# youngers2006/Dreamer

Hardware: AMD Instinct MI355X
Metric: imagined latent-steps/sec (B×H) at 64×64 CarRacing, 1/2/4/8 MI355X (higher is better)
Workload: dtype f32; 1 GPU; Dreamer.train_Agent() with AC_epochs=1 (replay sample + warm start S/2 + H-step imagination + actor-critic update), B=256/GPU S=64 H=15 64x64x3, precision=fp32 (north-star batch per GPU); global_batch=256, seq_len=64, horizon=15, parallelism=dp1, precision=fp32

## Files before the change

dreamer_amd/csrc/gemm.hip:

```cpp
#include <limits.h>
#include <stdlib.h>
#include <stdint.h>
#include <string.h>

#include "gemm.h"

#include <algorithm>

#define BK 32
#define LDS_K (BK + 2)

struct GemmBatch {
  GemmArgs p[4];
};

template <int BM, int BN>
__device__ __forceinline__ int dr_pack_tile(const GemmBatch& gb, int npack, int& z) {
  z = blockIdx.z;
  if (npack <= 0) return -2;
  int tot = 0;
  for (int i = 0; i < npack; ++i) tot += ((gb.p[i].M + BM - 1) / BM) * ((gb.p[i].N + BN - 1) / BN);
  int lt = dr_xcd_tile(blockIdx.x, tot);
  if (lt < 0) return -1;
  z = 0;
// ... 167 lines not shown
    if (!B_KN) {
      const int kk = tid & 31, nb = tid >> 5;
#pragma unroll
      for (int i = 0; i < NB; ++i) Bs[nb + 8 * i][kk] = rb[i];
    } else {
      const int nl = tid % BN, kb = tid / BN;
#pragma unroll
      for (int i = 0; i < NB; ++i) Bs[nl][kb + (256 / BN) * i] = rb[i];
    }
  };

  constexpr int WAVES_M = (BM >= 32) ? 2 : 1, WAVES_N = 4 / WAVES_M;
  constexpr int WTM = BM / WAVES_M, WTN = BN / WAVES_N;
  constexpr int FM = WTM / 16, FN = WTN / 16;
  static_assert(FM >= 1 && FN >= 1, "tile too small for 4 waves");
  const int wm0 = (wave / WAVES_N) * WTM, wn0 = (wave % WAVES_N) * WTN;
  f32x4 acc[FM][FN];
#pragma unroll
  for (int i = 0; i < FM; ++i)
#pragma unroll
    for (int j = 0; j < FN; ++j) acc[i][j] = (f32x4){0.f, 0.f, 0.f, 0.f};

  const int fr = lane & 15, fk = lane >> 4;
  load_tiles(0);
  for (int k0 = 0; k0 < K; k0 += BK) {
    __syncthreads();
    store_tiles();
    __syncthreads();
    if (k0 + BK < K) load_tiles(k0 + BK);
#pragma unroll
    for (int kk = 0; kk < BK; kk += 4) {
      float a[FM], b[FN];
#pragma unroll
      for (int i = 0; i < FM; ++i) a[i] = As[wm0 + i * 16 + fr][kk + fk];
#pragma unroll
      for (int j = 0; j < FN; ++j) b[j] = Bs[wn0 + j * 16 + fr][kk + fk];
#pragma unroll
      for (int i = 0; i < FM; ++i)
#pragma unroll
        for (int j = 0; j < FN; ++j) acc[i][j] = __builtin_amdgcn_mfma_f32_16x16x4f32(a[i], b[j], acc[i][j], 0, 0, 0);
    }
  }

#pragma unroll
  for (int i = 0; i < FM; ++i)
#pragma unroll
    for (int j = 0; j < FN; ++j)
#pragma unroll
      for (int r = 0; r < 4; ++r) {
        const int m = m0 + wm0 + i * 16 + fk * 4 + r;
        const int n = n0 + wn0 + j * 16 + fr;
        if (m >= M || n >= N) continue;
        float v = (g.alpha == 1.0f) ? acc[i][j][r] : g.alpha * acc[i][j][r];
        if (g.bias) v = v + g.bias[n];
        if (g.addend) v = v + g.addend[(long long)m * g.ld_add + n];
        if (g.act == 1) v = v / (1.0f + expf(-v));
        else if (g.act == 2) v = 1.0f / (1.0f + expf(-v));
        float* dst;
        if (g.out_conv) {
          const int hw = g.oh * g.ow;
          const int f = m / hw, pix = m - f * hw;
          dst = g.Y + ((long long)f * N + n) * hw + pix;
        } else if (n < g.nsplitY) {
          dst = g.Y + (long long)m * g.ldy + n;
        } else {
          dst = g.Y2 + (long long)m * g.ldy2 + (n - g.nsplitY);
        }
        if (g.accumulate) *dst = *dst + v;
        else *dst = v;
      }
}

#ifdef DR_PHASE_TIMING
__device__ long long dr_tbuf_gemm[1024 * DR_TS_SLOTS];
extern "C" int dr_debug_tbuf_gemm(long long* out, int n) {
  const int rc = (int)hipMemcpyFromSymbol(out, HIP_SYMBOL(dr_tbuf_gemm), (size_t)n * sizeof(long long));
  static long long zeros[1024 * DR_TS_SLOTS];
  return rc | (int)hipMemcpyToSymbol(HIP_SYMBOL(dr_tbuf_gemm), zeros, sizeof(zeros));
}
#endif
#define SK_LN_MAXF 33280
#define SK_LN_MAXK 2048
#define SK_STAGE 8

struct SkOps {
  const float *A, *A2, *W, *W2;
  int lda, lda2, ksA, ldb, ldb2, ksB, nsB, M, N, K;
};

template <bool B_KN, bool VEC>
__device__ __forceinline__ void skinny_load_b(const SkOps& o, int n, int kq, float (&b)[4]) {
  if (!B_KN && VEC) {
    const bool ok = (n < o.N) && (kq < o.K);
    float4 v = dr_ld4(o.W, ok ? (unsigned)(n * o.ldb + kq) : 0u);
    if (!ok) v = make_float4(0.f, 0.f, 0.f, 0.f);
    b[0] = v.x; b[1] = v.y; b[2] = v.z; b[3] = v.w;
    return;
  }
#pragma unroll
  for (int c = 0; c < 4; ++c) {
    const int k = kq + c;
    const bool ok = (n < o.N) && (k < o.K);
    float v;
    if (!B_KN) {
      v = dr_ld1(o.W, ok ? (unsigned)(n * o.ldb + k) : 0u);
    } else if (k >= o.ksB) {
      v = dr_ld1(o.W2, ok ? (unsigned)((k - o.ksB) * o.ldb2 + n) : 0u);
    } else if (n >= o.nsB) {
      v = dr_ld1(o.W2, ok ? (unsigned)(k * o.ldb2 + n - o.nsB) : 0u);
    } else {
      v = dr_ld1(o.W, ok ? (unsigned)(k * o.ldb + n) : 0u);
    }
    b[c] = ok ? v : 0.f;
  }
}

template <bool VEC>
__device__ __forceinline__ void skinny_load_a(const SkOps& o, int m, int k16, int kq, float (&a)[4]) {
  if (VEC) {
    const bool ok = (m < o.M) && (kq < o.K);
    float4 v;
    if (k16 + 16 <= o.ksA) {
      v = dr_ld4(o.A, ok ? (unsigned)(m * o.lda + kq) : 0u);
    } else if (k16 >= o.ksA) {
      v = dr_ld4(o.A2, ok ? (unsigned)(m * o.lda2 + kq - o.ksA) : 0u);
    } else {
      const float* src = (kq < o.ksA) ? o.A + (long long)m * o.lda + kq : o.A2 + (long long)m * o.lda2 + (kq - o.ksA);
      v = dr_ld4(ok ? src : o.A, 0u);
    }
    if (!ok) v = make_float4(0.f, 0.f, 0.f, 0.f);
    a[0] = v.x; a[1] = v.y; a[2] = v.z; a[3] = v.w;
  } else {
#pragma unroll
    for (int c = 0; c < 4; ++c) {
      const int k = kq + c;
      const bool ok = (m < o.M) && (k < o.K);
      float v;
      if (k < o.ksA) v = dr_ld1(o.A, ok ? (unsigned)(m * o.lda + k) : 0u);
      else v = dr_ld1(o.A2, ok ? (unsigned)(m * o.lda2 + k - o.ksA) : 0u);
      a[c] = ok ? v : 0.f;
    }
  }
}

__device__ __forceinline__ float epi_act(const GemmArgs& g, float v) {
  if (g.act == 1) return v / (1.0f + expf(-v));
  if (g.act == 2) return 1.0f / (1.0f + expf(-v));
  return v;
}

__device__ __noinline__ void gru_bwd_elem(const GruBwdEpi& e, int m, int j, float g) {
  const int Hd = e.Hd;
  const long long i = (long long)m * Hd + j;
  const float r = dr_g(e.r)[i], u = dr_g(e.u)[i], n = dr_g(e.n)[i], hn = dr_g(e.ghn)[i];
  const float hv = e.h ? dr_g(e.h)[(long long)m * e.ldh + j] : 0.0f;
  const float g_hmn = g * u;
  const float g_u = g * (hv - n);
  const float g_n = g + (-g_hmn);
  const float g_pn = g_n * (1.0f - n * n);
  const float g_r = g_pn * hn;
  const float g_hn = g_pn * r;
  const float g_pr = g_r * (1.0f - r) * r;
  const float g_pu = g_u * (1.0f - u) * u;
  DR_GLOBAL float* gib = dr_g(e.gi) + (long long)m * 3 * Hd;
  DR_GLOBAL float* ghb = dr_g(e.gh) + (long long)m * 3 * Hd;
  gib[j] = g_pr;
  gib[Hd + j] = g_pu;
  gib[2 * Hd + j] = g_pn;
  ghb[j] = g_pr;
  ghb[Hd + j] = g_pu;
  ghb[2 * Hd + j] = g_hn;
  if (e.gi16) {
    DR_GLOBAL unsigned short* gi16 = dr_g(e.gi16) + (long long)m * 3 * Hd;
    DR_GLOBAL unsigned short* gh16 = dr_g(e.gh16) + (long long)m * 3 * Hd;
    gi16[j] = __builtin_bit_cast(unsigned short, (__bf16)g_pr);
    gi16[Hd + j] = __builtin_bit_cast(unsigned short, (__bf16)g_pu);
    gi16[2 * Hd + j] = __builtin_bit_cast(unsigned short, (__bf16)g_pn);
    gh16[j] = __builtin_bit_cast(unsigned short, (__bf16)g_pr);
    gh16[Hd + j] = __builtin_bit_cast(unsigned short, (__bf16)g_pu);
    gh16[2 * Hd + j] = __builtin_bit_cast(unsigned short, (__bf16)g_hn);
  }
  DR_GLOBAL float* o = dr_g(e.ho) + (long long)m * e.ldo + j;
  *o = *o + g_hmn;
}

__device__ __forceinline__ void epilogue_store_b(const GemmArgs& g, int m, int n, float acc, float bias) {
  float v = (g.alpha == 1.0f) ? acc : g.alpha * acc;
  if (g.bias) v = v + bias;
  if (g.addend) v = v + dr_g(g.addend)[(long long)m * g.ld_add + n];
  v = epi_act(g, v);
  DR_GLOBAL float* dst;
  if (n < g.nsplitY) dst = dr_g(g.Y) + (long long)m * g.ldy + n;
  else dst = dr_g(g.Y2) + (long long)m * g.ldy2 + (n - g.nsplitY);
  const float fin = g.accumulate ? *dst + v : v;
  *dst = fin;
  if (g.gb.Hd > 0 && n < g.gb.Hd) gru_bwd_elem(g.gb, m, n, fin);
}

#define DR_SKW 8
template <int MT, int NT, int AMODE, bool B_KN, bool VEC, int EPI>
__global__ __launch_bounds__(64 * DR_SKW) void k_gemm_skinny(GemmBatch gb, int npack) {
  constexpr int NWAVE = DR_SKW, NTH = 64 * DR_SKW, FT = MT / 16, FN = NT / 16;
  __shared__ GemmArgs s_args;
  int pz;
  const int plt = dr_pack_tile<MT, NT>(gb, npack, pz);
  if (plt == -1) return;
  dr_stage_args(gb.p[pz], s_args, threadIdx.x);
  const GemmArgs& g = s_args;
  SkOps o;
  o.M = dr_uni(g.M); o.N = dr_uni(g.N); o.K = dr_uni(g.K);
  o.A = dr_uni(g.A); o.A2 = dr_uni(g.A2); o.W = dr_uni(g.W);
  o.lda = dr_uni((int)g.lda); o.lda2 = dr_uni((int)g.lda2); o.ksA = dr_uni(g.ksplitA); o.ldb = dr_uni((int)g.ldb);
  o.W2 = dr_uni(g.W2); o.ldb2 = dr_uni((int)g.ldb2); o.ksB = dr_uni(g.ksplitB); o.nsB = dr_uni(g.nsplitB);
  const int M = o.M, N = o.N, K = o.K;
  const int tiles_n = (N + NT - 1) / NT;
  const int tiles_m = (M + MT - 1) / MT;
  const int lt = plt >= 0 ? plt : dr_xcd_tile(blockIdx.x, tiles_m * tiles_n);
  if (lt < 0) return;
  const int tn = lt / tiles_m, tm = lt - tn * tiles_m;
  const int m0 = tm * MT, n0 = tn * NT;
  const int tid = threadIdx.x, wave = tid >> 6, lane = tid & 63;
  const int r = lane & 15, q = lane >> 4;
  DR_TS(dr_tbuf_gemm, 0);

  constexpr int RED = NWAVE * FT * FN * 4 * 64;
  extern __shared__ __attribute__((aligned(16))) float smem[];
  __shared__ float s_mean[MT], s_rstd[MT];
  __shared__ float s_out[MT][NT + 1];
  constexpr int NEPI = (FT * FN * 256 + NTH - 1) / NTH;
  float ebias[NEPI];
  {
    const float* bias = dr_uni(g.bias);
#pragma unroll
    for (int i = 0; i < NEPI; ++i) {
      const int x = tid + NTH * i;
      const int n = n0 + ((x >> 8) % FN) * 16 + (x & 15);
      const bool ok = bias && x < FT * FN * 256 && n < N;
      const float v = dr_ld1(ok ? bias : o.W, ok ? (unsigned)n : 0u);
      ebias[i] = ok ? v : 0.f;
    }
  }

  unsigned long long rng_seed = 0, rng_off = 0;
  if ((EPI == EPI_SAMPLE || EPI == EPI_ACTOR) && g.epi != EPI_NONE && !g.noise.q && !g.noise.eps && g.noise.rng) {
    rng_seed = g.noise.rng[0];
    rng_off = g.noise.rng[1];
  }
  const int kw = ((K + NWAVE * 16 - 1) / (NWAVE * 16)) * 16;
  const int kb = wave * kw;
  const int ke = min(K, kb + kw);

  const int KP = K + ((8 - (K & 15)) & 15);
  const int K4 = K >> 2;
  constexpr int RPW = MT / NWAVE;
  constexpr int BPW = (NT + NWAVE - 1) / NWAVE;
  constexpr int SV = (MT == 16) ? 4 : 1;
  float* a_out = dr_uni(g.a_out);
  const int ld_aout = dr_uni((int)g.ld_aout);
  const bool store_a = (a_out != nullptr) && (tn == 0);
  const bool staged = (AMODE == AM_LNSILU || AMODE == AM_LNBWD || AMODE == AM_STEBWD) && VEC && !B_KN &&
                     (K4 <= 64 * SV) &&
                     ((MT + NT) * KP <= SK_LN_MAXF);
  constexpr bool DUAL = FT * FN < 4;
  f32x4 acc[FT][FN], acc2[FT][FN];
#pragma unroll
  for (int t = 0; t < FT; ++t)
#pragma unroll
    for (int j = 0; j < FN; ++j) acc[t][j] = acc2[t][j] = (f32x4){0.f, 0.f, 0.f, 0.f};
  DR_TS(dr_tbuf_gemm, 1);
  if (staged) {
    float* sA = smem;
    float* sB = smem + MT * KP;
    constexpr int PRW = (AMODE == AM_LNBWD || AMODE == AM_STEBWD) ? RPW : 1;
    float4 xa[RPW][SV], xb[BPW][SV], gv[SV], bv[SV], xp[PRW][SV];
    const float* lg = dr_uni(g.ln_g);
    const float* lb = dr_uni(g.ln_b);
    const float* pre = dr_uni(g.pre);
    const int ld_pre = dr_uni((int)g.ld_pre);
#pragma unroll
    for (int i = 0; i < SV; ++i) {
      if (64 * i >= K4) break;
      const int k4 = lane + 64 * i, k = 4 * k4;
      const bool okk = k4 < K4;
#pragma unroll
      for (int rr = 0; rr < RPW; ++rr) {
        const int m = m0 + wave + NWAVE * rr;
        const bool ok = okk && m < M;
        const bool seg1 = k < o.ksA;
        const float* base = seg1 ? o.A : o.A2;
        const unsigned e = ok ? (unsigned)(seg1 ? m * o.lda + k : m * o.lda2 + k - o.ksA) : 0u;
        xa[rr][i] = dr_ld4(ok ? base : o.W, e);
        if (!ok) xa[rr][i] = make_float4(0.f, 0.f, 0.f, 0.f);
        if (AMODE == AM_LNBWD || AMODE == AM_STEBWD) {
          xp[rr][i] = dr_ld4(pre, ok ? (unsigned)(m * ld_pre + k) : 0u);
          if (!ok) xp[rr][i] = make_float4(0.f, 0.f, 0.f, 0.f);
        }
      }
#pragma unroll
      for (int jj = 0; jj < BPW; ++jj) {
        const int nl = wave + NWAVE * jj, n = n0 + nl;
        const bool ok = okk && nl < NT && n < N;
        xb[jj][i] = dr_ld4(o.W, ok ? (unsigned)(n * o.ldb + k) : 0u);
        if (!ok) xb[jj][i] = make_float4(0.f, 0.f, 0.f, 0.f);
      }
      if (AMODE == AM_LNSILU || AMODE == AM_LNBWD) {
        gv[i] = dr_ld4(lg, okk ? (unsigned)k : 0u);
        bv[i] = dr_ld4(lb, okk ? (unsigned)k : 0u);
      }
    }
    DR_TS(dr_tbuf_gemm, 2);
#pragma unroll
    for (int rr = 0; rr < RPW; ++rr) {
      const int ml = wave + NWAVE * rr, m = m0 + ml;
      if (AMODE == AM_LNSILU) {
        float sm = 0.f;
#pragma unroll
        for (int i = 0; i < SV; ++i) {
          if (64 * i >= K4) break;
          sm += (xa[rr][i].x + xa[rr][i].y) + (xa[rr][i].z + xa[rr][i].w);
        }
        const float mean = wave_sum(sm) / (float)K;
        float sq = 0.f;
#pragma unroll
        for (int i = 0; i < SV; ++i) {
          if (64 * i >= K4) break;
          if (lane + 64 * i < K4) {
            const float dx = xa[rr][i].x - mean, dy = xa[rr][i].y - mean;
            const float dz = xa[rr][i].z - mean, dw = xa[rr][i].w - mean;
            sq += (dx * dx + dy * dy) + (dz * dz + dw * dw);
          }
        }
        const float rstd = 1.0f / sqrtf(wave_sum(sq) / (float)K + 1e-5f);
#pragma unroll
        for (int i = 0; i < SV; ++i) {
          if (64 * i >= K4) break;
          float4& x = xa[rr][i];
          x.x = dr_silu_fast((x.x - mean) * rstd * gv[i].x + bv[i].x);
          x.y = dr_silu_fast((x.y - mean) * rstd * gv[i].y + bv[i].y);
          x.z = dr_silu_fast((x.z - mean) * rstd * gv[i].z + bv[i].z);
// ... 66 lines not shown
            gyp[c] = gxh;
            if (okk) {
              c1 += gxh;
              c2 += gxh * x_h;
            }
            if (save && okk) {
              dr_g(sgy)[(unsigned)(m * ld_sv + 4 * k4 + c)] = gyv;
              dr_g(sxh)[(unsigned)(m * ld_sv + 4 * k4 + c)] = x_h;
            }
          }
          xa[rr][i] = gy;
          xp[PR][i] = xh;
        }
        c1 = wave_sum(c1) / (float)K;
        c2 = wave_sum(c2) / (float)K;
#pragma unroll
        for (int i = 0; i < SV; ++i) {
          if (64 * i >= K4) break;
          float4& x = xa[rr][i];
          const float4& h = xp[PR][i];
          x.x = rstd * (x.x - c1 - h.x * c2);
          x.y = rstd * (x.y - c1 - h.y * c2);
          x.z = rstd * (x.z - c1 - h.z * c2);
          x.w = rstd * (x.w - c1 - h.w * c2);
          if (m >= M) x = make_float4(0.f, 0.f, 0.f, 0.f);
        }
      }
#pragma unroll
      for (int i = 0; i < SV; ++i) {
        if (64 * i >= K4) break;
        const int k4 = lane + 64 * i;
        if (k4 < K4) {
          *reinterpret_cast<float4*>(&sA[ml * KP + 4 * k4]) = xa[rr][i];
          if (store_a && m < M) dr_st4(a_out, (unsigned)(m * ld_aout + 4 * k4), xa[rr][i]);
        }
      }
    }
#pragma unroll
    for (int jj = 0; jj < BPW; ++jj) {
      const int nl = wave + NWAVE * jj;
      if (nl >= NT) break;
#pragma unroll
      for (int i = 0; i < SV; ++i) {
        if (64 * i >= K4) break;
        const int k4 = lane + 64 * i;
        if (k4 < K4) *reinterpret_cast<float4*>(&sB[nl * KP + 4 * k4]) = xb[jj][i];
      }
    }
    DR_TS(dr_tbuf_gemm, 6);
    __syncthreads();
    DR_TS(dr_tbuf_gemm, 3);
    for (int k16 = kb; k16 < ke; k16 += 16) {
      const int kq = k16 + 4 * q;
      const bool okq = kq < K;
      f32x4 (&ac)[FT][FN] = (DUAL && (((k16 - kb) >> 4) & 1)) ? acc2 : acc;
      float4 fa[FT], fb[FN];
#pragma unroll
      for (int t = 0; t < FT; ++t) {
        fa[t] = *reinterpret_cast<const float4*>(&sA[(t * 16 + r) * KP + (okq ? kq : 0)]);
        if (!okq) fa[t] = make_float4(0.f, 0.f, 0.f, 0.f);
      }
#pragma unroll
      for (int j = 0; j < FN; ++j) {
        fb[j] = *reinterpret_cast<const float4*>(&sB[(j * 16 + r) * KP + (okq ? kq : 0)]);
        if (!okq) fb[j] = make_float4(0.f, 0.f, 0.f, 0.f);
      }
#pragma unroll
      for (int t = 0; t < FT; ++t)
#pragma unroll
        for (int j = 0; j < FN; ++j) ac[t][j] = __builtin_amdgcn_mfma_f32_16x16x4f32(fa[t].x, fb[j].x, ac[t][j], 0, 0, 0);
#pragma unroll
      for (int t = 0; t < FT; ++t)
#pragma unroll
        for (int j = 0; j < FN; ++j) ac[t][j] = __builtin_amdgcn_mfma_f32_16x16x4f32(fa[t].y, fb[j].y, ac[t][j], 0, 0, 0);
#pragma unroll
      for (int t = 0; t < FT; ++t)
#pragma unroll
        for (int j = 0; j < FN; ++j) ac[t][j] = __builtin_amdgcn_mfma_f32_16x16x4f32(fa[t].z, fb[j].z, ac[t][j], 0, 0, 0);
#pragma unroll
      for (int t = 0; t < FT; ++t)
#pragma unroll
        for (int j = 0; j < FN; ++j) ac[t][j] = __builtin_amdgcn_mfma_f32_16x16x4f32(fa[t].w, fb[j].w, ac[t][j], 0, 0, 0);
    }
  } else {
    constexpr int PRE = (FT >= 4) ? 4 : 8;
    float bb[PRE][FN][4];
    float aa[PRE][FT][4];
    auto load_batch = [&](int kc) {
  #pragma unroll
      for (int p = 0; p < PRE; ++p) {
        const int k16 = kc + 16 * p;
        const int kq = k16 + 4 * q;
        const bool live = k16 < ke;
  #pragma unroll
        for (int j = 0; j < FN; ++j) {
          if (live) {
            skinny_load_b<B_KN, VEC>(o, n0 + j * 16 + r, kq, bb[p][j]);
          } else {
  #pragma unroll
            for (int c = 0; c < 4; ++c) bb[p][j][c] = 0.f;
          }
        }
        if (AMODE != AM_LNSILU) {
  #pragma unroll
          for (int t = 0; t < FT; ++t) {
            if (live) {
              skinny_load_a<VEC>(o, m0 + t * 16 + r, k16, kq, aa[p][t]);
            } else {
  #pragma unroll
              for (int c = 0; c < 4; ++c) aa[p][t][c] = 0.f;
            }
          }
        }
      }
    };
    if (kb < ke) load_batch(kb);

    constexpr int LNV = (MT == 16) ? 8 : 2;
    const bool ln_lds = (AMODE == AM_LNSILU) && VEC && (MT * KP <= SK_LN_MAXF) && (K4 <= 64 * LNV);
    if (AMODE == AM_LNSILU) {
      if (ln_lds) {
        const float* lg = dr_uni(g.ln_g);
        const float* lb = dr_uni(g.ln_b);
        float4 xv[RPW][LNV], gv[LNV], bv[LNV];
  #pragma unroll
        for (int i = 0; i < LNV; ++i) {
          if (64 * i >= K4) break;
          const int k4 = lane + 64 * i;
          const bool okk = k4 < K4;
          gv[i] = dr_ld4(lg, okk ? (unsigned)(4 * k4) : 0u);
          bv[i] = dr_ld4(lb, okk ? (unsigned)(4 * k4) : 0u);
  #pragma unroll
          for (int rr = 0; rr < RPW; ++rr) {
            const int m = m0 + wave + NWAVE * rr;
            const bool ok = okk && m < M;
            xv[rr][i] = dr_ld4(o.A, ok ? (unsigned)(m * o.lda + 4 * k4) : 0u);
            if (!ok) xv[rr][i] = make_float4(0.f, 0.f, 0.f, 0.f);
          }
        }
  #pragma unroll
        for (int rr = 0; rr < RPW; ++rr) {
          const int ml = wave + NWAVE * rr, m = m0 + ml;
          float sm = 0.f;
  #pragma unroll
          for (int i = 0; i < LNV; ++i) {
            if (64 * i >= K4) break;
            sm += (xv[rr][i].x + xv[rr][i].y) + (xv[rr][i].z + xv[rr][i].w);
          }
          const float mean = wave_sum(sm) / (float)K;
          float sq = 0.f;
  #pragma unroll
          for (int i = 0; i < LNV; ++i) {
            if (64 * i >= K4) break;
            if (lane + 64 * i < K4) {
              const float dx = xv[rr][i].x - mean, dy = xv[rr][i].y - mean;
              const float dz = xv[rr][i].z - mean, dw = xv[rr][i].w - mean;
              sq += (dx * dx + dy * dy) + (dz * dz + dw * dw);
            }
          }
          const float rstd = 1.0f / sqrtf(wave_sum(sq) / (float)K + 1e-5f);
  #pragma unroll
          for (int i = 0; i < LNV; ++i) {
            if (64 * i >= K4) break;
            const int k4 = lane + 64 * i;
            if (k4 < K4) {
              float4 y;
              y.x = dr_silu_fast((xv[rr][i].x - mean) * rstd * gv[i].x + bv[i].x);
// ... 42 lines not shown
          const bool live = k16 < ke;
  #pragma unroll
          for (int t = 0; t < FT; ++t) {
            const int ml = t * 16 + r, m = m0 + ml;
            if (!live) {
  #pragma unroll
              for (int c = 0; c < 4; ++c) aa[p][t][c] = 0.f;
            } else if (ln_lds) {
              if (m < M && kq < K) {
                const float4 v = *reinterpret_cast<const float4*>(&smem[ml * KP + kq]);
                aa[p][t][0] = v.x; aa[p][t][1] = v.y; aa[p][t][2] = v.z; aa[p][t][3] = v.w;
              } else {
                aa[p][t][0] = aa[p][t][1] = aa[p][t][2] = aa[p][t][3] = 0.f;
              }
            } else {
              skinny_load_a<VEC>(o, m, k16, kq, aa[p][t]);
            }
          }
        }
      }
  #pragma unroll
      for (int p = 0; p < PRE; ++p) {
        if (kc + 16 * p >= ke) break;
        const int kq = kc + 16 * p + 4 * q;
  #pragma unroll
        for (int t = 0; t < FT; ++t) {
          const int ml = t * 16 + r, m = m0 + ml;
          if (AMODE == AM_LNSILU && !ln_lds) {
            const float mean = s_mean[ml], rstd = s_rstd[ml];
  #pragma unroll
            for (int c = 0; c < 4; ++c) {
              const int k = kq + c;
              if (m < M && k < K) {
                float x = (aa[p][t][c] - mean) * rstd;
                x = x * dr_ld1(lg, (unsigned)k) + dr_ld1(lb, (unsigned)k);
                aa[p][t][c] = dr_silu_fast(x);
              }
            }
          }
          if (store_a && m < M && !(AMODE == AM_LNSILU && ln_lds)) {
  #pragma unroll
            for (int c = 0; c < 4; ++c)
              if (kq + c < K) dr_g(a_out)[(unsigned)(m * ld_aout + kq + c)] = aa[p][t][c];
          }
        }
        f32x4 (&ac)[FT][FN] = (DUAL && (p & 1)) ? acc2 : acc;
  #pragma unroll
        for (int c = 0; c < 4; ++c)
  #pragma unroll
          for (int t = 0; t < FT; ++t)
  #pragma unroll
            for (int j = 0; j < FN; ++j)
              ac[t][j] = __builtin_amdgcn_mfma_f32_16x16x4f32(aa[p][t][c], bb[p][j][c], ac[t][j], 0, 0, 0);
      }
    }
  }
  if (DUAL) {
#pragma unroll
    for (int t = 0; t < FT; ++t)
#pragma unroll
      for (int j = 0; j < FN; ++j) acc[t][j] += acc2[t][j];
  }
  DR_TS(dr_tbuf_gemm, 4);
  if (staged || AMODE == AM_LNSILU) __syncthreads();
#pragma unroll
  for (int t = 0; t < FT; ++t)
#pragma unroll
    for (int j = 0; j < FN; ++j)
#pragma unroll
      for (int e = 0; e < 4; ++e) smem[(((wave * FT + t) * FN + j) * 4 + e) * 64 + lane] = acc[t][j][e];
  __syncthreads();
  DR_TS(dr_tbuf_gemm, 5);
#pragma unroll
  for (int i = 0; i < NEPI; ++i) {
    const int x = tid + NTH * i;
    if (x >= FT * FN * 256) break;
    const int l = x & 63, e = (x >> 6) & 3, tj = x >> 8;
    float v = 0.f;
#pragma unroll
    for (int w = 0; w < NWAVE; ++w) v += smem[((w * FT * FN + tj) * 4 + e) * 64 + l];
    const int t = tj / FN, j = tj - t * FN;
    const int ml = t * 16 + 4 * (l >> 4) + e, nl = j * 16 + (l & 15);
    const int m = m0 + ml, n = n0 + nl;
    if (EPI == EPI_NONE || g.epi == EPI_NONE) {
      if (m < M && n < N) epilogue_store_b(g, m, n, v, ebias[i]);
    } else {
      if (m < M && n < N) {
        float y = v + ebias[i];
        if (g.Y) dr_g(g.Y)[(long long)m * g.ldy + n] = y;
        s_out[ml][nl] = y;
      }
    }
  }
  if (EPI == EPI_SAMPLE) {
    __syncthreads();
    const int C = g.C;
    int W = 1;
    while (W < C) W <<= 1;
    const int gpr = NT / C;
    const int npairs = MT * gpr;
    const int per_wave = 64 / W;
    for (int pbase = wave * per_wave; pbase < npairs; pbase += NWAVE * per_wave) {
      const int pidx = pbase + lane / W, c = lane % W;
      const bool valid = pidx < npairs;
      const int ml = valid ? pidx / gpr : 0, gl = valid ? pidx - ml * gpr : 0;
      const int m = m0 + ml, grp = (n0 / C) + gl;
      const bool act = valid && c < C && m < M && (n0 + gl * C + c) < N;
      const float x = act ? s_out[ml][gl * C + c] : -INFINITY;
      const float mx = group_max(x, W);
      const float ex = act ? expf(x - mx) : 0.0f;
      const float se = group_sum(ex, W);
      const float p = ex / se;
      const float pu = act ? (0.99f * p + g.unimix) : 0.0f;
      const float sp = group_sum(pu, W);
      const float ph = pu / sp;
      float qv = 1.0f;
      const int Rg = g.R;
      if (act) {
        if (g.noise.q) qv = dr_g(g.noise.q)[((long long)g.step * M * Rg + (long long)m * Rg + grp) * C + c];
        else qv = dr_exp1_k(rng_seed, rng_off, (uint32_t)(g.noise.stream + g.step), (uint32_t)(g.noise.row0 + m),
                            (uint32_t)(grp * C + c));
      }
      float best = act ? ph / qv : -INFINITY;
      int bi = act ? c : 0x7fffffff;
      group_argmax(best, bi, W);
      if (act) {
        dr_g(g.z_out)[(long long)m * g.ldz + grp * C + c] = (c == bi) ? ((1.0f + pu) - pu) : 0.0f;
        if (g.soft_out) dr_g(g.soft_out)[(long long)m * g.ld_soft + grp * C + c] = p;
        if (g.idx_out && c == 0) dr_g(g.idx_out)[m * Rg + grp] = bi;
        if (g.zval_out && c == bi) dr_g(g.zval_out)[m * Rg + grp] = (1.0f + pu) - pu;
      }
    }
    DR_TS(dr_tbuf_gemm, 7);
  } else if (EPI == EPI_ACTOR && g.epi == EPI_ACTOR) {
    __syncthreads();
    const int A = g.na;
    for (int x = tid; x < MT * A; x += NTH) {
      const int ml = x / A, i = x - ml * A, m = m0 + ml;
      if (m >= M) continue;
      const float muv = s_out[ml][i];
      const float lr = s_out[ml][A + i];
      const float ls = fminf(fmaxf(lr, -5.0f), 2.0f);
      const float sg = dr_softplus(ls) + 1e-3f;
      float av;
      if (g.det) {
        av = tanhf(muv);
      } else {
        float e;
        if (g.noise.eps) e = dr_g(g.noise.eps)[((long long)g.step * M + m) * A + i];
        else e = dr_normal_k(rng_seed, rng_off, (uint32_t)(g.noise.stream + g.step), (uint32_t)(g.noise.row0 + m),
                             (uint32_t)i);
        if (g.eps_save) dr_g(g.eps_save)[(long long)m * A + i] = e;
        av = tanhf(muv + e * sg);
      }
      if (g.act_out) dr_g(g.act_out)[(long long)m * g.ld_act + i] = av;
      if (g.mu_out) dr_g(g.mu_out)[(long long)m * g.ld_mu + i] = muv;
      if (g.sig_out) dr_g(g.sig_out)[(long long)m * g.ld_sig + i] = sg;
      if (g.ls_save) dr_g(g.ls_save)[(long long)m * g.ld_ls + i] = lr;
    }
  }
}

__device__ __forceinline__ void epilogue_store(const GemmArgs& g, int m, int n, float acc) {
  epilogue_store_b(g, m, n, acc, g.bias ? dr_g(g.bias)[n] : 0.f);
}

#define LS_MT 16
// ... 782 lines not shown
        }
      }
#define DR_WK3(PA, PB, X)                        \
  _Pragma("unroll") for (int i = 0; i < FM; ++i) _Pragma("unroll") for (int j = 0; j < FN; ++j) acc[X][i][j] = \
      wk_mfma(rb[u][PB][j], a[PA][i], acc[X][i][j]);
      if constexpr (NTP == 3) {
        DR_WK3(2 % NTP, 0, 0)
        DR_WK3(1 % NTP, 1 % NTP, 0)
        DR_WK3(0, 2 % NTP, 0)
        DR_WK3(1 % NTP, 0, 0)
        DR_WK3(0, 1 % NTP, 0)
      }
      DR_WK3(0, 0, 0)
#undef DR_WK3
      load(min(c + D, clast), u);
    }
  }
  {
#pragma unroll
    for (int i = 0; i < FM; ++i)
#pragma unroll
      for (int j = 0; j < FN; ++j) {
        const f32x4 v = acc[0][i][j];
#pragma unroll
        for (int e = 0; e < 4; ++e) red[wave][(i * FN + j) * 4 + e][lane] = v[e];
      }
  }
  __syncthreads();
#pragma unroll
  for (int ii = 0; ii < NEPI; ++ii) {
    const int x = tid + NTH * ii;
    if (x >= NT4) break;
    const int l = x & 63, e = (x >> 6) & 3, tj = x >> 8;
    float v = 0.f;
#pragma unroll
    for (int w = 0; w < NW; ++w) v += red[w][tj * 4 + e][l];
    const int t = tj / FN, j = tj - t * FN;
    const int m = m0 + t * 16 + (l & 15), n = n0 + j * 16 + 4 * (l >> 4) + e;
    if (m >= M || n >= N) continue;
    epilogue_store_b(g, m, n, v, ebias[ii]);
  }
}

__global__ __launch_bounds__(256) void k_splitk_finish(GemmBatch gb, int splits) {
  __shared__ GemmArgs s_args;
  dr_stage_args(gb.p[blockIdx.z], s_args, threadIdx.x);
  const GemmArgs& g = s_args;
  const long long MN = (long long)g.M * g.N;
  const long long i = (long long)blockIdx.x * 256 + threadIdx.x;
  if (i >= MN) return;
  float v = 0.f;
  for (int sp = 0; sp < splits; ++sp) v += dr_g(g.splitk_ws)[sp * MN + i];
  const int m = (int)(i / g.N), n = (int)(i - (long long)m * g.N);
  epilogue_store(g, m, n, v);
}

static bool aligned16(const void* p) { return ((uintptr_t)p & 15) == 0; }

static bool skinny_vec_ok(const GemmArgs& g, bool b_kn) {
  if (g.K % 4 != 0 || !aligned16(g.A) || g.lda % 4 != 0) return false;
  if (g.ksplitA < g.K && (!aligned16(g.A2) || g.lda2 % 4 != 0 || g.ksplitA % 4 != 0)) return false;
  if (!b_kn && (!aligned16(g.W) || g.ldb % 4 != 0)) return false;
  return true;
}

static bool skinny_offsets_ok(const GemmArgs& g, bool b_kn) {
  const long long lim = 1LL << 30;
  if ((long long)g.M * g.lda >= lim || (long long)g.M * g.lda2 >= lim) return false;
  if ((b_kn ? (long long)g.K * g.ldb : (long long)g.N * g.ldb) >= lim) return false;
  if (g.W2 && (long long)(g.K + g.N) * g.ldb2 >= lim) return false;
  if (g.a_out && (long long)g.M * g.ld_aout >= lim) return false;
  return true;
}

template <int MT, int NT, int AMODE, bool B_KN>
static size_t skinny_lds_floats(const GemmBatch& gb, int count, bool vec) {
  const size_t red = (size_t)DR_SKW * (MT / 16) * (NT / 16) * 4 * 64;
  size_t need = red;
  if (!vec) return need;
  for (int i = 0; i < count; ++i) {
    const size_t K = gb.p[i].K, KP = K + ((8 - (K & 15)) & 15);
    const size_t staged = (size_t)(MT + NT) * KP, rows = (size_t)MT * KP;
    if ((AMODE == AM_LNSILU || AMODE == AM_LNBWD || AMODE == AM_STEBWD) && !B_KN &&
        K / 4 <= 64 * (MT == 16 ? 4 : 1) &&
        staged <= SK_LN_MAXF)
      need = std::max(need, staged);
    else if (AMODE == AM_LNSILU && rows <= SK_LN_MAXF && K / 4 <= 64 * (MT == 16 ? 8 : 2))
      need = std::max(need, rows);
  }
  return need;
}

template <int MT, int NT, int AMODE, bool B_KN, int EPI>
static void launch_skinny(const GemmBatch& gb, int count, bool vec, hipStream_t s) {
  int maxt = 0;
  for (int i = 0; i < count; ++i) {
    const int t = dr_cdiv(gb.p[i].M, MT) * dr_cdiv(gb.p[i].N, NT);
    maxt = t > maxt ? t : maxt;
  }
  if (maxt == 0) return;
  const size_t lds = skinny_lds_floats<MT, NT, AMODE, B_KN>(gb, count, vec) * sizeof(float);
  if (lds > 64 * 1024) {
    static const bool raised = [] {
      (void)hipFuncSetAttribute((const void*)k_gemm_skinny<MT, NT, AMODE, B_KN, true, EPI>,
                                hipFuncAttributeMaxDynamicSharedMemorySize, 150 * 1024);
      (void)hipFuncSetAttribute((const void*)k_gemm_skinny<MT, NT, AMODE, B_KN, false, EPI>,
                                hipFuncAttributeMaxDynamicSharedMemorySize, 150 * 1024);
      return true;
    }();
    (void)raised;
  }
  const int npack = count > 1 ? count : 0;
  const dim3 grid(dr_xcd_grid(npack ? pack_tiles(gb, count, MT, NT) : maxt), 1, npack ? 1 : count);
  if (vec)
    hipLaunchKernelGGL((k_gemm_skinny<MT, NT, AMODE, B_KN, true, EPI>), grid, dim3(64 * DR_SKW), lds, s, gb, npack);
  else
    hipLaunchKernelGGL((k_gemm_skinny<MT, NT, AMODE, B_KN, false, EPI>), grid, dim3(64 * DR_SKW), lds, s, gb, npack);
}



bool gemm_bwd_rows16(const GemmArgs* p, int count) {
  int maxM = 0, t16 = 0;
  for (int i = 0; i < count; ++i) {
    maxM = std::max(maxM, p[i].M);
    t16 += dr_cdiv(p[i].M, 16) * dr_cdiv(p[i].N, 16);
  }
  return maxM <= 64 || (maxM <= 4096 && t16 <= 640);
}

template <int AMODE, bool B_KN>
static bool try_skinny(const GemmBatch& gb, int count, hipStream_t s) {
  int maxM = 0, epi = EPI_NONE;
  bool vec = true;
  for (int i = 0; i < count; ++i) {
    const GemmArgs& g = gb.p[i];
    if (g.out_conv) return false;
    if ((g.epi == EPI_SAMPLE) != (gb.p[0].epi == EPI_SAMPLE)) return false;
    if (g.epi != EPI_NONE) epi = g.epi;
    maxM = g.M > maxM ? g.M : maxM;
    if (!skinny_offsets_ok(g, B_KN)) return false;
    vec = vec && skinny_vec_ok(g, B_KN);
  }
  if (maxM > (epi == EPI_NONE ? (1 << 20) : 4096)) return false;
  if (maxM > 64 && (AMODE == AM_PLAIN || AMODE == AM_LNSILU || AMODE == AM_LNBWD || AMODE == AM_STEBWD)) {
    int t16 = 0;
    for (int i = 0; i < count; ++i) t16 += dr_cdiv(gb.p[i].M, 16) * dr_cdiv(gb.p[i].N, epi == EPI_SAMPLE ? 32 : 16);
    if (t16 <= 640) maxM = 64;
  }
  int tiles16 = 0;
  for (int i = 0; i < count; ++i)
    tiles16 += dr_cdiv(gb.p[i].M, maxM > 64 ? 64 : 16) * dr_cdiv(gb.p[i].N, 16);
  bool wide = maxM <= 64 && tiles16 > 256;
  if (AMODE == AM_LNBWD || AMODE == AM_STEBWD) {
    const int mt = maxM > 64 ? 64 : 16;
    for (int i = 0; i < count; ++i) {
      const int K = gb.p[i].K, KP = K + ((8 - (K & 15)) & 15);
      const int nt = (epi == EPI_SAMPLE || wide) ? 32 : 16;
      if ((mt + nt) * KP > SK_LN_MAXF && nt == 32 && epi != EPI_SAMPLE) wide = false;
      if ((mt + (wide || epi == EPI_SAMPLE ? 32 : 16)) * KP > SK_LN_MAXF || K / 4 > 64 * (mt == 16 ? 4 : 1) || !vec)
        return false;
    }
  }
  if (epi == EPI_SAMPLE) {
    if (maxM > 64) launch_skinny<64, 32, AMODE, B_KN, EPI_SAMPLE>(gb, count, vec, s);
    else launch_skinny<16, 32, AMODE, B_KN, EPI_SAMPLE>(gb, count, vec, s);
  } else if (epi == EPI_ACTOR) {
    if (maxM > 64) launch_skinny<64, 16, AMODE, B_KN, EPI_ACTOR>(gb, count, vec, s);
    else launch_skinny<16, 16, AMODE, B_KN, EPI_ACTOR>(gb, count, vec, s);
  } else {
    if (maxM > 64) launch_skinny<64, 16, AMODE, B_KN, EPI_NONE>(gb, count, vec, s);
    else if (wide) launch_skinny<16, 32, AMODE, B_KN, EPI_NONE>(gb, count, vec, s);
    else launch_skinny<16, 16, AMODE, B_KN, EPI_NONE>(gb, count, vec, s);
  }
  return true;
}

template <int BM, int BN, int AMODE, bool A_KM, bool B_KN>
static void launch_tile(const GemmBatch& gb, int count, hipStream_t s) {
  int maxt = 0;
  for (int i = 0; i < count; ++i) {
    const int t = dr_cdiv(gb.p[i].M, BM) * dr_cdiv(gb.p[i].N, BN);
    maxt = t > maxt ? t : maxt;
  }
  if (maxt == 0) return;
  hipLaunchKernelGGL((k_gemm<BM, BN, AMODE, A_KM, B_KN>), dim3(maxt, 1, count), dim3(256), 0, s, gb);
}

#define MLP2_KMAX 208
#define MLP2_NC 128
struct Mlp2Batch {
  Mlp2Args p[3];
};

__device__ __forceinline__ float4 mlp2_ln_silu(float4 x, bool ok, int K, const float* gam, const float* bet, int k) {
  const float mean = wave_sum(ok ? (x.x + x.y) + (x.z + x.w) : 0.f) / (float)K;
  float sq = 0.f;
  if (ok) {
    const float dx = x.x - mean, dy = x.y - mean, dz = x.z - mean, dw = x.w - mean;
    sq = (dx * dx + dy * dy) + (dz * dz + dw * dw);
  }
  const float rstd = 1.0f / sqrtf(wave_sum(sq) / (float)K + 1e-5f);
  if (!ok) return make_float4(0.f, 0.f, 0.f, 0.f);
  const float4 gv = dr_ld4(gam, (unsigned)k), bv = dr_ld4(bet, (unsigned)k);
  return make_float4(dr_silu_fast((x.x - mean) * rstd * gv.x + bv.x), dr_silu_fast((x.y - mean) * rstd * gv.y + bv.y),
                     dr_silu_fast((x.z - mean) * rstd * gv.z + bv.z), dr_silu_fast((x.w - mean) * rstd * gv.w + bv.w));
}

#define MLP2_KS (MLP2_KMAX / 16)
__device__ __forceinline__ void mlp2_wload(float4 (&wv)[MLP2_KS], const float* W, int ldw, int n, bool nok, int K,
                                           int q) {
  const int ks = (K + 15) >> 4;
#pragma unroll
  for (int s = 0; s < MLP2_KS; ++s) {
    const int k = 16 * s + 4 * q;
    const bool ok = s < ks && nok && k < K;
    wv[s] = dr_ld4(W, ok ? (unsigned)(n * ldw + k) : 0u);
    if (!ok) wv[s] = make_float4(0.f, 0.f, 0.f, 0.f);
  }
}
template <int LP>
__device__ __forceinline__ f32x4 mlp2_tile(const float (*ys)[LP], const float4 (&wv)[MLP2_KS], int K, int r, int q) {
  const int ks = (K + 15) >> 4;
  f32x4 c[4];
#pragma unroll
  for (int j = 0; j < 4; ++j) c[j] = (f32x4){0.f, 0.f, 0.f, 0.f};
#pragma unroll
  for (int s = 0; s < MLP2_KS; ++s) {
    if (s < ks) {
      const float4 a = *reinterpret_cast<const float4*>(&ys[r][16 * s + 4 * q]);
      c[s & 3] = __builtin_amdgcn_mfma_f32_16x16x4f32(a.x, wv[s].x, c[s & 3], 0, 0, 0);
      c[s & 3] = __builtin_amdgcn_mfma_f32_16x16x4f32(a.y, wv[s].y, c[s & 3], 0, 0, 0);
      c[s & 3] = __builtin_amdgcn_mfma_f32_16x16x4f32(a.z, wv[s].z, c[s & 3], 0, 0, 0);
      c[s & 3] = __builtin_amdgcn_mfma_f32_16x16x4f32(a.w, wv[s].w, c[s & 3], 0, 0, 0);
    }
  }
  f32x4 o;
#pragma unroll
  for (int e = 0; e < 4; ++e) o[e] = (c[0][e] + c[1][e]) + (c[2][e] + c[3][e]);
  return o;
}

__global__ __launch_bounds__(512) void k_mlp2_tail(Mlp2Batch mb) {
  __shared__ Mlp2Args s_a;
  dr_stage_args(mb.p[blockIdx.z], s_a, threadIdx.x);
  const Mlp2Args& a = s_a;
  const GemmArgs& g = a.e;
  const int M = dr_uni(a.M), K1 = dr_uni(a.K1), K2 = dr_uni(a.K2), N = dr_uni(g.N);
  const int n0 = blockIdx.x * MLP2_NC, m0 = blockIdx.y * 16;
  if (n0 >= N || m0 >= M) return;
  const int tid = threadIdx.x, wave = tid >> 6, lane = tid & 63;
  const int r = lane & 15, q = lane >> 4;
  constexpr int LP = MLP2_KMAX + 8;
  __shared__ __attribute__((aligned(16))) float ys[16][LP];
  __shared__ __attribute__((aligned(16))) float hs[16][LP];
// ... 611 lines not shown
```

Measured before the change: 618,200 imagined latent-steps/s.

## Prefetch GRU-backward epilogue operands and add 16x48 skinny tile for LN-backward

In the LN-backward skinny GEMM, the epilogue operands (accumulate destination, GRU gate values r/u/n/ghn, hidden state, output gradient) are now loaded into registers before the main loop, so their latency overlaps with compute instead of stalling the store phase. The non-inlined per-element GRU backward helper is split so the prefetched values can be reused, with a guard for the case where the output aliases the destination. A 16x48 tile variant is chosen when 32-wide tiles would give between 256 and 512 tiles but 48-wide tiles fit in 256. The unstaged fallback path is compiled out for LN-backward. This raises register pressure and adds another template instantiation.

After: 630,300 imagined latent-steps/s, median of 6. +2.0%, better.

```diff
diff --git a/dreamer_amd/csrc/gemm.hip b/dreamer_amd/csrc/gemm.hip
--- a/dreamer_amd/csrc/gemm.hip
+++ b/dreamer_amd/csrc/gemm.hip
@@ -273,6 +273,7 @@
 #define SK_LN_MAXF 33280
 #define SK_LN_MAXK 2048
 #define SK_STAGE 8
+constexpr __host__ __device__ int sk_stage_vecs(int mt, int nt) { return (mt == 16 && nt <= 32) ? 4 : 1; }
 
 struct SkOps {
   const float *A, *A2, *W, *W2;
@@ -340,11 +341,9 @@
   return v;
 }
 
-__device__ __noinline__ void gru_bwd_elem(const GruBwdEpi& e, int m, int j, float g) {
+__device__ __forceinline__ void gru_bwd_apply(const GruBwdEpi& e, int m, int j, float g, float r, float u, float n,
+                                              float hn, float hv, float o_old) {
   const int Hd = e.Hd;
-  const long long i = (long long)m * Hd + j;
-  const float r = dr_g(e.r)[i], u = dr_g(e.u)[i], n = dr_g(e.n)[i], hn = dr_g(e.ghn)[i];
-  const float hv = e.h ? dr_g(e.h)[(long long)m * e.ldh + j] : 0.0f;
   const float g_hmn = g * u;
   const float g_u = g * (hv - n);
   const float g_n = g + (-g_hmn);
@@ -371,8 +370,14 @@
     gh16[Hd + j] = __builtin_bit_cast(unsigned short, (__bf16)g_pu);
     gh16[2 * Hd + j] = __builtin_bit_cast(unsigned short, (__bf16)g_hn);
   }
-  DR_GLOBAL float* o = dr_g(e.ho) + (long long)m * e.ldo + j;
-  *o = *o + g_hmn;
+  dr_g(e.ho)[(long long)m * e.ldo + j] = o_old + g_hmn;
+}
+
+__device__ __noinline__ void gru_bwd_elem(const GruBwdEpi& e, int m, int j, float g) {
+  const long long i = (long long)m * e.Hd + j;
+  const float r = dr_g(e.r)[i], u = dr_g(e.u)[i], n = dr_g(e.n)[i], hn = dr_g(e.ghn)[i];
+  const float hv = e.h ? dr_g(e.h)[(long long)m * e.ldh + j] : 0.0f;
+  gru_bwd_apply(e, m, j, g, r, u, n, hn, hv, dr_g(e.ho)[(long long)m * e.ldo + j]);
 }
 
 __device__ __forceinline__ void epilogue_store_b(const GemmArgs& g, int m, int n, float acc, float bias) {
@@ -386,6 +391,44 @@
   const float fin = g.accumulate ? *dst + v : v;
   *dst = fin;
   if (g.gb.Hd > 0 && n < g.gb.Hd) gru_bwd_elem(g.gb, m, n, fin);
+}
+
+struct SkEpiPf {
+  float dst, r, u, n, hn, h, o;
+};
+__device__ __forceinline__ DR_GLOBAL float* sk_epi_dst(const GemmArgs& g, int m, int n) {
+  if (n < g.nsplitY) return dr_g(g.Y) + (long long)m * g.ldy + n;
+  return dr_g(g.Y2) + (long long)m * g.ldy2 + (n - g.nsplitY);
+}
+__device__ __forceinline__ SkEpiPf sk_epi_prefetch(const GemmArgs& g, int m, int n, bool ok) {
+  SkEpiPf p = {0.f, 0.f, 0.f, 0.f, 0.f, 0.f, 0.f};
+  if (!ok) return p;
+  if (g.accumulate) p.dst = *sk_epi_dst(g, m, n);
+  const GruBwdEpi& e = g.gb;
+  if (e.Hd > 0 && n < e.Hd) {
+    const long long i = (long long)m * e.Hd + n;
+    p.r = dr_g(e.r)[i];
+    p.u = dr_g(e.u)[i];
+    p.n = dr_g(e.n)[i];
+    p.hn = dr_g(e.ghn)[i];
+    if (e.h) p.h = dr_g(e.h)[(long long)m * e.ldh + n];
+    p.o = dr_g(e.ho)[(long long)m * e.ldo + n];
+  }
+  return p;
+}
+__device__ __forceinline__ void epilogue_store_pf(const GemmArgs& g, int m, int n, float acc, float bias,
+                                                  const SkEpiPf& p) {
+  float v = (g.alpha == 1.0f) ? acc : g.alpha * acc;
+  if (g.bias) v = v + bias;
+  if (g.addend) v = v + dr_g(g.addend)[(long long)m * g.ld_add + n];
+  v = epi_act(g, v);
+  DR_GLOBAL float* dst = sk_epi_dst(g, m, n);
+  const float fin = g.accumulate ? p.dst + v : v;
+  *dst = fin;
+  if (g.gb.Hd > 0 && n < g.gb.Hd) {
+    const DR_GLOBAL float* o = dr_g(g.gb.ho) + (long long)m * g.gb.ldo + n;
+    gru_bwd_apply(g.gb, m, n, fin, p.r, p.u, p.n, p.hn, p.h, o == dst ? fin : p.o);
+  }
 }
 
 #define DR_SKW 8
@@ -431,6 +474,18 @@
       ebias[i] = ok ? v : 0.f;
     }
   }
+  constexpr bool PFE = (AMODE == AM_LNBWD) && (EPI == EPI_NONE);
+  SkEpiPf pf[PFE ? NEPI : 1];
+  if (PFE) {
+#pragma unroll
+    for (int i = 0; i < NEPI; ++i) {
+      const int x = tid + NTH * i;
+      const int l = x & 63, e = (x >> 6) & 3, tj = x >> 8;
+      const int t = tj / FN, j = tj - t * FN;
+      const int m = m0 + t * 16 + 4 * (l >> 4) + e, n = n0 + j * 16 + (l & 15);
+      pf[i] = sk_epi_prefetch(g, m, n, x < FT * FN * 256 && m < M && n < N);
+    }
+  }
 
   unsigned long long rng_seed = 0, rng_off = 0;
   if ((EPI == EPI_SAMPLE || EPI == EPI_ACTOR) && g.epi != EPI_NONE && !g.noise.q && !g.noise.eps && g.noise.rng) {
@@ -445,7 +500,7 @@
   const int K4 = K >> 2;
   constexpr int RPW = MT / NWAVE;
   constexpr int BPW = (NT + NWAVE - 1) / NWAVE;
-  constexpr int SV = (MT == 16) ? 4 : 1;
+  constexpr int SV = sk_stage_vecs(MT, NT);
   float* a_out = dr_uni(g.a_out);
   const int ld_aout = dr_uni((int)g.ld_aout);
   const bool store_a = (a_out != nullptr) && (tn == 0);
@@ -678,7 +733,7 @@
 #pragma unroll
         for (int j = 0; j < FN; ++j) ac[t][j] = __builtin_amdgcn_mfma_f32_16x16x4f32(fa[t].w, fb[j].w, ac[t][j], 0, 0, 0);
     }
-  } else {
+  } else if (AMODE != AM_LNBWD) {
     constexpr int PRE = (FT >= 4) ? 4 : 8;
     float bb[PRE][FN][4];
     float aa[PRE][FT][4];
@@ -887,7 +942,9 @@
     const int t = tj / FN, j = tj - t * FN;
     const int ml = t * 16 + 4 * (l >> 4) + e, nl = j * 16 + (l & 15);
     const int m = m0 + ml, n = n0 + nl;
-    if (EPI == EPI_NONE || g.epi == EPI_NONE) {
+    if (PFE) {
+      if (m < M && n < N) epilogue_store_pf(g, m, n, v, ebias[i], pf[i]);
+    } else if (EPI == EPI_NONE || g.epi == EPI_NONE) {
       if (m < M && n < N) epilogue_store_b(g, m, n, v, ebias[i]);
     } else {
       if (m < M && n < N) {
@@ -1836,7 +1893,7 @@
     const size_t K = gb.p[i].K, KP = K + ((8 - (K & 15)) & 15);
     const size_t staged = (size_t)(MT + NT) * KP, rows = (size_t)MT * KP;
     if ((AMODE == AM_LNSILU || AMODE == AM_LNBWD || AMODE == AM_STEBWD) && !B_KN &&
-        K / 4 <= 64 * (MT == 16 ? 4 : 1) &&
+        K / 4 <= 64 * (size_t)sk_stage_vecs(MT, NT) &&
         staged <= SK_LN_MAXF)
       need = std::max(need, staged);
     else if (AMODE == AM_LNSILU && rows <= SK_LN_MAXF && K / 4 <= 64 * (MT == 16 ? 8 : 2))
@@ -1906,6 +1963,18 @@
   for (int i = 0; i < count; ++i)
     tiles16 += dr_cdiv(gb.p[i].M, maxM > 64 ? 64 : 16) * dr_cdiv(gb.p[i].N, 16);
   bool wide = maxM <= 64 && tiles16 > 256;
+  bool wide48 = false;
+  if (AMODE == AM_LNBWD && epi == EPI_NONE && wide && vec) {
+    int t32 = 0, t48 = 0;
+    bool fits = true;
+    for (int i = 0; i < count; ++i) {
+      const int K = gb.p[i].K, KP = K + ((8 - (K & 15)) & 15);
+      t32 += dr_cdiv(gb.p[i].M, 16) * dr_cdiv(gb.p[i].N, 32);
+      t48 += dr_cdiv(gb.p[i].M, 16) * dr_cdiv(gb.p[i].N, 48);
+      fits = fits && (16 + 48) * KP <= SK_LN_MAXF && K / 4 <= 64 * sk_stage_vecs(16, 48);
+    }
+    wide48 = fits && t32 > 256 && t32 < 512 && t48 <= 256;
+  }
   if (AMODE == AM_LNBWD || AMODE == AM_STEBWD) {
     const int mt = maxM > 64 ? 64 : 16;
     for (int i = 0; i < count; ++i) {
@@ -1923,8 +1992,11 @@
     if (maxM > 64) launch_skinny<64, 16, AMODE, B_KN, EPI_ACTOR>(gb, count, vec, s);
     else launch_skinny<16, 16, AMODE, B_KN, EPI_ACTOR>(gb, count, vec, s);
   } else {
-    if (maxM > 64) launch_skinny<64, 16, AMODE, B_KN, EPI_NONE>(gb, count, vec, s);
-    else if (wide) launch_skinny<16, 32, AMODE, B_KN, EPI_NONE>(gb, count, vec, s);
+    if (maxM > 64) {
+      launch_skinny<64, 16, AMODE, B_KN, EPI_NONE>(gb, count, vec, s);
+    } else if (wide48) {
+      if constexpr (AMODE == AM_LNBWD) launch_skinny<16, 48, AM_LNBWD, B_KN, EPI_NONE>(gb, count, vec, s);
+    } else if (wide) launch_skinny<16, 32, AMODE, B_KN, EPI_NONE>(gb, count, vec, s);
     else launch_skinny<16, 16, AMODE, B_KN, EPI_NONE>(gb, count, vec, s);
   }
   return true;
```
